# fnzhan/EMLight

Measured on AMD Instinct MI355X. Metric: training images/sec (regression step: DenseNet-BC fwd + Sinkhorn loss + bwd + Adam), higher is better.
Workload: dtype f32; 1 GPU; RegressionNetwork train step, BASELINE configs[1]; per_gpu_batch=64, global_batch=64, anchors=128, parallelism=single

## Files before the change

### emlight_amd/csrc/dense_bwd.hip

```cpp
#include "eml_common.h"
#include "eml_dropout.h"

#include <cstdint>
#include <cstdlib>
#include <type_traits>

namespace {

using f32x4 = __attribute__((ext_vector_type(4))) float;

__device__ __forceinline__ f32x4 mfma16(float a, float b, f32x4 c) {
  return __builtin_amdgcn_mfma_f32_16x16x4f32(a, b, c, 0, 0, 0);
}
__device__ __forceinline__ float f4c(const float4& v, int t) { return t == 0 ? v.x : t == 1 ? v.y : t == 2 ? v.z : v.w; }
__device__ __forceinline__ double shfl_xor_d(double v, int m) { return __shfl_xor(v, m, 64); }

constexpr int kTH = 8, kTW = 32, kHH = kTH + 2, kHW = kTW + 2;

constexpr int kPSG = 14;
constexpr int kBD = 512;
constexpr int kGRows = 2;
constexpr int kGPass = kHH / kGRows;

template <bool FUSE, bool WIDE, int TH, bool DROP = false>
// ... 1719 lines not shown
          const float4 c4 = *reinterpret_cast<const float4*>(co_l + 2 * Ko + ch);
          float4 dz[MT];
#pragma unroll
          for (int m = 0; m < MT; ++m) {
            dz[m].x = fmaf(a4.x, ry[m].x, fmaf(b4.x, rz[m].x, c4.x));
            dz[m].y = fmaf(a4.y, ry[m].y, fmaf(b4.y, rz[m].y, c4.y));
            dz[m].z = fmaf(a4.z, ry[m].z, fmaf(b4.z, rz[m].z, c4.z));
            dz[m].w = fmaf(a4.w, ry[m].w, fmaf(b4.w, rz[m].w, c4.w));
          }
          group_step(jo, dz);
        }
      }
      if constexpr (MASKED && !ACC) {
        float l1n[NCH][4];
        float4 skn[NCH];
#pragma unroll
        for (int n = 0; n < NCH; ++n) {
          skn[n] = *reinterpret_cast<const float4*>(vec_l + 16 * min(nt0 + n, nnt - 1) + 4 * kk);
#pragma unroll
          for (int g = 0; g < 4; ++g) l1n[n][g] = 0.f;
        }
        const int piece = lane & 7;
        const bool col_ok = nt0 + (piece >> 2) < nnt;
#pragma unroll
        for (int m = 0; m < MT; ++m) {
#pragma unroll
          for (int sub = 0; sub < 4; ++sub) {
#pragma unroll
            for (int n = 0; n < NCH; ++n) {
              const unsigned b = pv[m] ? mk[m][n] >> (4 * sub) : 0u;
              const float d0 = (b & 1u) ? 0.25f * acc[m][n][0] : 0.f, d1 = (b & 2u) ? 0.25f * acc[m][n][1] : 0.f;
              const float d2 = (b & 4u) ? 0.25f * acc[m][n][2] : 0.f, d3 = (b & 8u) ? 0.25f * acc[m][n][3] : 0.f;
              *reinterpret_cast<f32x4*>(stg + r * 36 + 16 * n + 4 * kk) = f32x4{skn[n].x * d0, skn[n].y * d1, skn[n].z * d2, skn[n].w * d3};
              if (nt0 + n < nnt) {
                l1n[n][0] += d0;
                l1n[n][1] += d1;
                l1n[n][2] += d2;
                l1n[n][3] += d3;
              }
            }
            __builtin_amdgcn_fence(__ATOMIC_RELEASE, "wavefront");
            __builtin_amdgcn_wave_barrier();
            __builtin_amdgcn_fence(__ATOMIC_ACQUIRE, "wavefront");
            const size_t suboff = ((size_t)(sub >> 1) * Win + (sub & 1)) * (size_t)ldg + 16 * nt0 + 4 * piece;
#pragma unroll
            for (int h = 0; h < 2; ++h) {
              const f32x4 v = *reinterpret_cast<const f32x4*>(stg + ((lane >> 3) + 8 * h) * 36 + 4 * piece);
              if (pvx[m][h] && col_ok) *reinterpret_cast<f32x4*>(Gd + pinx[m][h] * ldg + suboff) = v;
            }
            __builtin_amdgcn_fence(__ATOMIC_RELEASE, "wavefront");
            __builtin_amdgcn_wave_barrier();
            __builtin_amdgcn_fence(__ATOMIC_ACQUIRE, "wavefront");
          }
        }
#pragma unroll
        for (int n = 0; n < NCH; ++n) {
          if (nt0 + n < nnt) {
            const int k4 = 16 * (nt0 + n) + 4 * kk;
#pragma unroll
            for (int g = 0; g < 4; ++g) {
              const float t1 = eml::row16_sum(l1n[n][g]);
              if (r == 0) my[2 * (k4 + g)] += (double)t1;
            }
          }
        }
      } else {
#pragma unroll
      for (int n = 0; n < NCH; ++n) {
        const int nt = nt0 + n;
        if (nt < nnt) {
          const int k4 = 16 * nt + 4 * kk;
          const float4 sk = *reinterpret_cast<const float4*>(vec_l + k4);
          const float4 tk = *reinterpret_cast<const float4*>(vec_l + Kp + k4);
          const float4 mu = *reinterpret_cast<const float4*>(vec_l + 2 * Kp + k4);
          const float4 is = *reinterpret_cast<const float4*>(vec_l + 3 * Kp + k4);
          float l1[4] = {0.f, 0.f, 0.f, 0.f}, l2[4] = {0.f, 0.f, 0.f, 0.f};
#pragma unroll
          for (int m = 0; m < MT; ++m) {
            const float da0 = 0.25f * acc[m][n][0], da1 = 0.25f * acc[m][n][1];
            const float da2 = 0.25f * acc[m][n][2], da3 = 0.25f * acc[m][n][3];
#pragma unroll
            for (int sub = 0; sub < 4; ++sub) {
              float4 g = make_float4(0.f, 0.f, 0.f, 0.f);
              if constexpr (ACC) g = gs[m][n][sub];
              float d0, d1, d2, d3;
              float4 x = make_float4(0.f, 0.f, 0.f, 0.f);
              if constexpr (MASKED) {
                const unsigned b = pv[m] ? mk[m][n] >> (4 * sub) : 0u;
                d0 = (b & 1u) ? da0 : 0.f;
                d1 = (b & 2u) ? da1 : 0.f;
                d2 = (b & 4u) ? da2 : 0.f;
                d3 = (b & 8u) ? da3 : 0.f;
              } else {
                x = xv[m][n][sub];
                d0 = (pv[m] && fmaf(x.x, sk.x, tk.x) > 0.f) ? da0 : 0.f;
                d1 = (pv[m] && fmaf(x.y, sk.y, tk.y) > 0.f) ? da1 : 0.f;
                d2 = (pv[m] && fmaf(x.z, sk.z, tk.z) > 0.f) ? da2 : 0.f;
                d3 = (pv[m] && fmaf(x.w, sk.w, tk.w) > 0.f) ? da3 : 0.f;
              }
              g.x = fmaf(sk.x, d0, g.x);
              g.y = fmaf(sk.y, d1, g.y);
              g.z = fmaf(sk.z, d2, g.z);
              g.w = fmaf(sk.w, d3, g.w);
              if (pv[m]) {
                const size_t pi = pin[m] + (sub >> 1) * (size_t)Win + (sub & 1);
                *reinterpret_cast<float4*>(Gd + pi * ldg + k4) = g;
              }
              l1[0] += d0;
              l1[1] += d1;
              l1[2] += d2;
              l1[3] += d3;
              if constexpr (!MASKED) {
                l2[0] = fmaf(d0, (x.x - mu.x) * is.x, l2[0]);
                l2[1] = fmaf(d1, (x.y - mu.y) * is.y, l2[1]);
                l2[2] = fmaf(d2, (x.z - mu.z) * is.z, l2[2]);
                l2[3] = fmaf(d3, (x.w - mu.w) * is.w, l2[3]);
              }
            }
          }
#pragma unroll
          for (int g = 0; g < 4; ++g) {
            l1[g] = eml::row16_sum(l1[g]);
            if constexpr (!MASKED) l2[g] = eml::row16_sum(l2[g]);
            if (r == 0) {
              my[2 * (k4 + g)] += (double)l1[g];
              if constexpr (!MASKED) my[2 * (k4 + g) + 1] += (double)l2[g];
            }
          }
        }
      }
      }
    }
  }
  __syncthreads();
  for (int e = tid; e < Kp * 2; e += 256)
    partials[(size_t)blockIdx.x * Kp * 2 + e] =
        (sacc[e] + sacc[(size_t)Kp * 2 + e]) + (sacc[(size_t)2 * Kp * 2 + e] + sacc[(size_t)3 * Kp * 2 + e]);
}

struct BwdLayer {
  const float* DZ;
  const float* Zr;
  const float* cA;
  const float* cB;
  const float* cC;
  const float* Wd;
  const float* scale1;
  const float* shift1;
  double* partials;
  int Kp;
};

template <int NL, int MT , bool RAW = false ,
          bool MASKED = false, bool TOP = false>
__global__ __launch_bounds__(256, 2) void conv1x1_bwd_data_multi_kernel(BwdLayer L0, BwdLayer L1,
                                                                        const float* __restrict__ X, int ldx,
                                                                        const float* __restrict__ mean,
                                                                        const float* __restrict__ istd, int P,
                                                                        int k_lo, int k_hi, float* __restrict__ Gd,
                                                                        int ldg, int KpMax,
                                                                        const unsigned long long* __restrict__ M0,
                                                                        const unsigned long long* __restrict__ M1,
                                                                        float* __restrict__ Top) {
  extern __shared__ __attribute__((aligned(16))) float smem[];
  double* sacc = reinterpret_cast<double*>(smem);
  float* vec_l = reinterpret_cast<float*>(sacc + (size_t)NL * 4 * KpMax * 2);
  const int tid = threadIdx.x, lane = tid & 63, wave = tid >> 6;
  const int r = lane & 15, kk = lane >> 4;
  const BwdLayer Ls[2] = {L0, L1};
  for (int e = tid; e < NL * 4 * KpMax * 2; e += 256) sacc[e] = 0.0;
  for (int e = tid; e < KpMax; e += 256) {
    vec_l[e] = MASKED ? 0.f : mean[e];
    vec_l[KpMax + e] = MASKED ? 0.f : istd[e];
#pragma unroll
    for (int j = 0; j < NL; ++j) {
      vec_l[(2 + 2 * j) * KpMax + e] = e < Ls[j].Kp ? Ls[j].scale1[e] : 0.f;
      vec_l[(3 + 2 * j) * KpMax + e] = e < Ls[j].Kp ? Ls[j].shift1[e] : 0.f;
    }
  }
  __syncthreads();
  constexpr int TP = 64 * MT;
  const int ntiles = (P + TP - 1) / TP;
  const int nt_lo = k_lo >> 4, nt_hi = (k_hi + 15) >> 4;
  constexpr int NCH = 2;

  float4 wq[2][3][NCH];
  auto load_w = [&](int j, int nt0, float4 (&dst)[3][NCH]) {
    const int nnt = Ls[j].Kp >> 4;
#pragma unroll
    for (int jo = 0; jo < 3; ++jo)
#pragma unroll
      for (int n = 0; n < NCH; ++n) {
        const int nt = min(nt0 + n, nnt - 1);
        dst[jo][n] = *reinterpret_cast<const float4*>(Ls[j].Wd + ((((size_t)nt * 3 + jo) * 4 + kk) * 16 + r) * 4);
      }
  };
  load_w(0, nt_lo, wq[0]);
  int wsel = 0;

  for (int tile = blockIdx.x; tile < ntiles; tile += gridDim.x) {
    const int p0 = tile * TP + wave * 16 * MT;
    long prow[MT];
    bool pv[MT];
#pragma unroll
    for (int m = 0; m < MT; ++m) {
      pv[m] = p0 + 16 * m + r < P;
      prow[m] = min(p0 + 16 * m + r, P - 1);
    }
    unsigned long long pvb[MT];
#pragma unroll
    for (int m = 0; m < MT; ++m) pvb[m] = MASKED ? __ballot(pv[m]) : 0ull;
    float4 dz[NL][3][MT];
#pragma unroll
    for (int j = 0; j < NL; ++j)
#pragma unroll
      for (int jo = 0; jo < 3; ++jo) {
        const int ch = 16 * jo + 4 * kk;
        if constexpr (RAW) {
#pragma unroll
          for (int m = 0; m < MT; ++m) dz[j][jo][m] = *reinterpret_cast<const float4*>(Ls[j].DZ + prow[m] * 48 + ch);
        } else {
          const float4 a4 = *reinterpret_cast<const float4*>(Ls[j].cA + ch);
          const float4 b4 = *reinterpret_cast<const float4*>(Ls[j].cB + ch);
          const float4 c4 = *reinterpret_cast<const float4*>(Ls[j].cC + ch);
#pragma unroll
          for (int m = 0; m < MT; ++m) {
            const float4 dy = *reinterpret_cast<const float4*>(Ls[j].DZ + prow[m] * 48 + ch);
            const float4 zr = *reinterpret_cast<const float4*>(Ls[j].Zr + prow[m] * 48 + ch);
            dz[j][jo][m].x = fmaf(a4.x, dy.x, fmaf(b4.x, zr.x, c4.x));
            dz[j][jo][m].y = fmaf(a4.y, dy.y, fmaf(b4.y, zr.y, c4.y));
            dz[j][jo][m].z = fmaf(a4.z, dy.z, fmaf(b4.z, zr.z, c4.z));
            dz[j][jo][m].w = fmaf(a4.w, dy.w, fmaf(b4.w, zr.w, c4.w));
          }
        }
      }
    for (int nt0 = nt_lo; nt0 < nt_hi; nt0 += NCH) {
      float4 gs[MT][NCH], xv[MT][NCH];
#pragma unroll
      for (int n = 0; n < NCH; ++n) {
        const int k4 = 16 * min(nt0 + n, nt_hi - 1) + 4 * kk;
        const int k4l = (k4 + 3 >= k_lo && k4 < k_hi) ? k4 : (k_lo & ~3);
#pragma unroll
        for (int m = 0; m < MT; ++m) {
          gs[m][n] = *reinterpret_cast<const float4*>(Gd + prow[m] * ldg + k4l);
          if constexpr (!MASKED) xv[m][n] = *reinterpret_cast<const float4*>(X + prow[m] * ldx + k4l);
        }
      }
      const int nt_next = nt0 + NCH < nt_hi ? nt0 + NCH : nt_lo;
#pragma unroll
      for (int j = 0; j < NL; ++j) {
        const int nnt = Ls[j].Kp >> 4;
        unsigned long long mk[MT][NCH][4];
        if constexpr (MASKED) {
          const unsigned long long* __restrict__ Mj = j == 0 ? M0 : M1;
#pragma unroll
          for (int m = 0; m < MT; ++m)
#pragma unroll
            for (int n = 0; n < NCH; ++n) {
              const size_t wi =
                  ((size_t)__builtin_amdgcn_readfirstlane((p0 >> 4) + m) * nnt + min(nt0 + n, nnt - 1)) * 4;
#pragma unroll
              for (int g = 0; g < 4; ++g) mk[m][n][g] = Mj[wi + g];
            }
        }
        const int cur = NL == 2 ? j : wsel;
        if (j + 1 < NL)
          load_w(j + 1, nt0, wq[cur ^ 1]);
        else
          load_w(0, nt_next, wq[cur ^ 1]);
        __builtin_amdgcn_sched_barrier(0);
        f32x4 acc[MT][NCH];
#pragma unroll
        for (int m = 0; m < MT; ++m)
#pragma unroll
          for (int n = 0; n < NCH; ++n) acc[m][n] = f32x4{0.f, 0.f, 0.f, 0.f};
#pragma unroll
        for (int jo = 0; jo < 3; ++jo)
#pragma unroll
          for (int t = 0; t < 4; ++t)
#pragma unroll
            for (int n = 0; n < NCH; ++n)
#pragma unroll
              for (int m = 0; m < MT; ++m) acc[m][n] = mfma16(f4c(wq[cur][jo][n], t), f4c(dz[j][jo][m], t), acc[m][n]);
        if (NL == 1) wsel ^= 1;
        double* my = sacc + ((size_t)(j * 4 + wave) * KpMax) * 2;
#pragma unroll
        for (int n = 0; n < NCH; ++n) {
          const int nt = nt0 + n;
          if (nt < nnt && nt < nt_hi) {
            const int k4 = 16 * nt + 4 * kk;
            const float4 mu = *reinterpret_cast<const float4*>(vec_l + k4);
            const float4 is = *reinterpret_cast<const float4*>(vec_l + KpMax + k4);
            const float4 sk = *reinterpret_cast<const float4*>(vec_l + (2 + 2 * j) * KpMax + k4);
            const float4 tk = *reinterpret_cast<const float4*>(vec_l + (3 + 2 * j) * KpMax + k4);
            const bool in0 = k4 + 0 >= k_lo && k4 + 0 < k_hi, in1 = k4 + 1 >= k_lo && k4 + 1 < k_hi;
            const bool in2 = k4 + 2 >= k_lo && k4 + 2 < k_hi, in3 = k4 + 3 >= k_lo && k4 + 3 < k_hi;
            unsigned long long inb[4] = {0ull, 0ull, 0ull, 0ull};
            if constexpr (MASKED) {
              inb[0] = __ballot(in0);
              inb[1] = __ballot(in1);
              inb[2] = __ballot(in2);
              inb[3] = __ballot(in3);
            }
            float l1[4] = {0.f, 0.f, 0.f, 0.f}, l2[4] = {0.f, 0.f, 0.f, 0.f};
#pragma unroll
            for (int m = 0; m < MT; ++m) {
              float d0, d1, d2, d3;
              if constexpr (MASKED) {
                d0 = __builtin_amdgcn_inverse_ballot_w64(mk[m][n][0] & pvb[m] & inb[0]) ? acc[m][n][0] : 0.f;
                d1 = __builtin_amdgcn_inverse_ballot_w64(mk[m][n][1] & pvb[m] & inb[1]) ? acc[m][n][1] : 0.f;
                d2 = __builtin_amdgcn_inverse_ballot_w64(mk[m][n][2] & pvb[m] & inb[2]) ? acc[m][n][2] : 0.f;
                d3 = __builtin_amdgcn_inverse_ballot_w64(mk[m][n][3] & pvb[m] & inb[3]) ? acc[m][n][3] : 0.f;
              } else {
                const float4 x = xv[m][n];
                d0 = (pv[m] && in0 && fmaf(x.x, sk.x, tk.x) > 0.f) ? acc[m][n][0] : 0.f;
                d1 = (pv[m] && in1 && fmaf(x.y, sk.y, tk.y) > 0.f) ? acc[m][n][1] : 0.f;
                d2 = (pv[m] && in2 && fmaf(x.z, sk.z, tk.z) > 0.f) ? acc[m][n][2] : 0.f;
                d3 = (pv[m] && in3 && fmaf(x.w, sk.w, tk.w) > 0.f) ? acc[m][n][3] : 0.f;
                l2[0] = fmaf(d0, (x.x - mu.x) * is.x, l2[0]);
                l2[1] = fmaf(d1, (x.y - mu.y) * is.y, l2[1]);
                l2[2] = fmaf(d2, (x.z - mu.z) * is.z, l2[2]);
                l2[3] = fmaf(d3, (x.w - mu.w) * is.w, l2[3]);
              }
              gs[m][n].x = fmaf(sk.x, d0, gs[m][n].x);
              gs[m][n].y = fmaf(sk.y, d1, gs[m][n].y);
              gs[m][n].z = fmaf(sk.z, d2, gs[m][n].z);
              gs[m][n].w = fmaf(sk.w, d3, gs[m][n].w);
              l1[0] += d0;
              l1[1] += d1;
              l1[2] += d2;
              l1[3] += d3;
            }
#pragma unroll
            for (int g = 0; g < 4; ++g) {
              l1[g] = eml::row16_sum(l1[g]);
              if constexpr (!MASKED) l2[g] = eml::row16_sum(l2[g]);
              if (r == 0) {
                my[2 * (k4 + g)] += (double)l1[g];
                if constexpr (!MASKED) my[2 * (k4 + g) + 1] += (double)l2[g];
              }
            }
          }
        }
      }
#pragma unroll
      for (int n = 0; n < NCH; ++n) {
        const int nt = nt0 + n;
        if (nt < nt_hi) {
          const int k4 = 16 * nt + 4 * kk;
          const bool act = k4 + 3 >= k_lo && k4 < k_hi;
          if constexpr (TOP) {
            const int t = k4 - (k_hi - 24);
            float* cdst = Top + (t >= 12 ? (size_t)P * 12 + (t - 12) : (size_t)max(t, 0));
#pragma unroll
            for (int m = 0; m < MT; ++m) {
              float* dst = t >= 0 ? cdst + prow[m] * 12 : Gd + prow[m] * ldg + k4;
              if (pv[m] && act) *reinterpret_cast<float4*>(dst) = gs[m][n];
            }
          } else {
#pragma unroll
            for (int m = 0; m < MT; ++m) {
              if (pv[m] && act) *reinterpret_cast<float4*>(Gd + prow[m] * ldg + k4) = gs[m][n];
            }
          }
        }
      }
    }
  }
  __syncthreads();
#pragma unroll
  for (int j = 0; j < NL; ++j) {
    const int Kp = Ls[j].Kp;
    const double* base = sacc + (size_t)j * 4 * KpMax * 2;
    for (int e = tid; e < Kp * 2; e += 256)
      Ls[j].partials[(size_t)blockIdx.x * Kp * 2 + e] = (base[e] + base[(size_t)KpMax * 2 + e]) +
                                                        (base[(size_t)2 * KpMax * 2 + e] + base[(size_t)3 * KpMax * 2 + e]);
  }
}

template <int MT>
__global__ __launch_bounds__(256, 2) void conv1x1_bwd_narrow_kernel(
    const float* __restrict__ DZ, const float* __restrict__ W1 , int Cin, int k_lo,
    const float* __restrict__ X, int ldx, const float* __restrict__ scale1, const float* __restrict__ shift1,
    const float* __restrict__ mean, const float* __restrict__ istd, int P, const float* __restrict__ Gd, int ldg,
    float* __restrict__ N12, double* __restrict__ partials , int Kp) {
  __shared__ double red[4][12][2];
  const int tid = threadIdx.x, lane = tid & 63, wave = tid >> 6;
  const int r = lane & 15, kk = lane >> 4;
  float aw[3][4];
#pragma unroll
  for (int jo = 0; jo < 3; ++jo)
#pragma unroll
    for (int t = 0; t < 4; ++t) aw[jo][t] = r < 12 ? W1[(size_t)(16 * jo + 4 * kk + t) * Cin + k_lo + r] : 0.f;
  const bool cv = kk < 3;
  const int cq = k_lo + 4 * (cv ? kk : 2);
  float sk[4], tk[4], mu[4], is[4];
#pragma unroll
  for (int g = 0; g < 4; ++g) {
    sk[g] = scale1[cq + g];
    tk[g] = shift1[cq + g];
    mu[g] = mean[cq + g];
    is[g] = istd[cq + g];
  }
  double s1[4] = {0.0, 0.0, 0.0, 0.0}, s2[4] = {0.0, 0.0, 0.0, 0.0};
  constexpr int TP = 64 * MT;
  const int ntiles = (P + TP - 1) / TP;
  for (int tile = blockIdx.x; tile < ntiles; tile += gridDim.x) {
    const int p0 = tile * TP + wave * 16 * MT;
    size_t prow[MT];
    bool pv[MT];
    float4 dz[MT][3];
    float2 xa[MT], xb[MT], ga[MT], gb[MT];
#pragma unroll
    for (int m = 0; m < MT; ++m) {
      pv[m] = p0 + 16 * m + r < P;
      prow[m] = (size_t)min(p0 + 16 * m + r, P - 1);
#pragma unroll
      for (int jo = 0; jo < 3; ++jo) dz[m][jo] = *reinterpret_cast<const float4*>(DZ + prow[m] * 48 + 16 * jo + 4 * kk);
      xa[m] = *reinterpret_cast<const float2*>(X + prow[m] * ldx + cq);
      xb[m] = *reinterpret_cast<const float2*>(X + prow[m] * ldx + cq + 2);
      ga[m] = *reinterpret_cast<const float2*>(Gd + prow[m] * ldg + cq);
      gb[m] = *reinterpret_cast<const float2*>(Gd + prow[m] * ldg + cq + 2);
    }
    f32x4 acc[MT];
#pragma unroll
    for (int m = 0; m < MT; ++m) acc[m] = f32x4{0.f, 0.f, 0.f, 0.f};
#pragma unroll
    for (int jo = 0; jo < 3; ++jo)
#pragma unroll
      for (int t = 0; t < 4; ++t)
#pragma unroll
        for (int m = 0; m < MT; ++m) acc[m] = mfma16(aw[jo][t], f4c(dz[m][jo], t), acc[m]);
#pragma unroll
    for (int m = 0; m < MT; ++m) {
      const float x[4] = {xa[m].x, xa[m].y, xb[m].x, xb[m].y};
      const float gold[4] = {ga[m].x, ga[m].y, gb[m].x, gb[m].y};
      float o[4];
#pragma unroll
      for (int g = 0; g < 4; ++g) {
        const float d = (pv[m] && cv && fmaf(x[g], sk[g], tk[g]) > 0.f) ? acc[m][g] : 0.f;
        o[g] = fmaf(sk[g], d, gold[g]);
        s1[g] += (double)d;
        s2[g] += (double)(d * ((x[g] - mu[g]) * is[g]));
      }
      if (pv[m] && cv) *reinterpret_cast<float4*>(N12 + prow[m] * 12 + 4 * kk) = make_float4(o[0], o[1], o[2], o[3]);
    }
  }
#pragma unroll
  for (int g = 0; g < 4; ++g) {
#pragma unroll
    for (int o = 1; o < 16; o <<= 1) {
      s1[g] += shfl_xor_d(s1[g], o);
      s2[g] += shfl_xor_d(s2[g], o);
    }
    if (r == 0 && cv) {
      red[wave][4 * kk + g][0] = s1[g];
      red[wave][4 * kk + g][1] = s2[g];
    }
  }
  __syncthreads();
  if (tid < 24) {
    const int c = tid >> 1, e = tid & 1;
    partials[((size_t)blockIdx.x * Kp + k_lo + c) * 2 + e] = (red[0][c][e] + red[1][c][e]) + (red[2][c][e] + red[3][c][e]);
  }
}

__global__ void permute_w1_bwd_kernel(const float* __restrict__ W, int Cout, int Cin, int Kp, int Ko,
                                      float* __restrict__ Wd) {
  const size_t total = (size_t)Kp * Ko;
  for (size_t e = (size_t)blockIdx.x * blockDim.x + threadIdx.x; e < total; e += (size_t)gridDim.x * blockDim.x) {
    const int t = (int)(e & 3), col = (int)((e >> 2) & 15), kk = (int)((e >> 6) & 3);
    const size_t rest = e >> 8;
    const int jo = (int)(rest % (Ko >> 4)), nt = (int)(rest / (Ko >> 4));
    const int o = 16 * jo + 4 * kk + t, k = 16 * nt + col;
    Wd[e] = (o < Cout && k < Cin) ? W[(size_t)o * Cin + k] : 0.f;
  }
}

__global__ __launch_bounds__(256) void grad_materialize_kernel(float* __restrict__ Gd, int ldg,
                                                               const float* __restrict__ X, int ldx,
                                                               const float* __restrict__ sB,
                                                               const float* __restrict__ sC, int c0, int n, size_t P) {
  const int nh = n >> 1;
  const size_t total = P * nh;
  for (size_t e = (size_t)blockIdx.x * 256 + threadIdx.x; e < total; e += (size_t)gridDim.x * 256) {
    const size_t p = e / nh;
    const int c = c0 + 2 * (int)(e - p * nh);
    const float2 x = *reinterpret_cast<const float2*>(X + p * ldx + c);
    float2* gp = reinterpret_cast<float2*>(Gd + p * ldg + c);
    float2 g = *gp;
    g.x += fmaf(sB[c], x.x, sC[c]);
    g.y += fmaf(sB[c + 1], x.y, sC[c + 1]);
    *gp = g;
// ... 695 lines not shown
extern "C" int eml_dense_conv1x1_bwd_weight_f32(const float* X, int ldx, long P, int Hin, int Win, int pool, int Kp,
                                                int Cin, const float* scale1, const float* shift1, const float* DY,
                                                int ld_dy, const float* Zr, int ld_z, const float* cA, const float* cB,
                                                const float* cC, int Cout, float* partial, float* dW, int grid,
                                                float* dz_out, const float* W1, int k_lo, const float* G, int ldg,
                                                float* N12, double* partials_n, eml_stream_t stream) {
  if (dz_out && (Cout != 48 || pool))
    return eml::fail(EML_EINVAL, "eml_dense_conv1x1_bwd_weight_f32: dz_out is for dense layers (Cout == 48, no pool)");
  if (N12 && (Cout != 48 || pool || !W1 || !G || !partials_n || k_lo < 0 || (k_lo & 1) || k_lo + 12 > Cin || (ldg & 1) ||
              (ldg != 12 && k_lo + 12 > ldg)))
    return eml::fail(EML_EINVAL, "eml_dense_conv1x1_bwd_weight_f32: fused narrow pass needs a dense layer, W1, G, partials_n "
                                 "and an even k_lo with k_lo + 12 <= Cin (k_lo=%d, Cin=%d)", k_lo, Cin);
  if (!X || !scale1 || !shift1 || !DY || !Zr || !cA || !cB || !cC || !partial || !dW || P < 1 || grid < 1 || Kp < 32 ||
      (Kp & 15) || Cin > Kp || Cout < 1)
    return eml::fail(EML_EINVAL, "eml_dense_conv1x1_bwd_weight_f32: bad arguments");
  const int nchunks = (Cout + 47) / 48;
  for (int ch = 0; ch < nchunks; ++ch) {
    const int n0 = ch * 48, nv = (Cout - n0 < 48) ? Cout - n0 : 48;
    int n_load = ((ld_dy < ld_z ? ld_dy : ld_z) - n0) & ~3;
    if (n_load > 48) n_load = 48;
    if (n_load < nv) return eml::fail(EML_EINVAL, "eml_dense_conv1x1_bwd_weight_f32: DY/Zr rows narrower than Cout");
    const NarrowArgs na{W1, G, N12, partials_n, Cin, k_lo, ldg};
    static const int vec_env = [] { const char* v = getenv("EML_W1_VEC"); return v ? atoi(v) : 0; }();
    const bool vec4 = !pool && (ldx & 3) == 0 && (reinterpret_cast<uintptr_t>(X) & 15) == 0 &&
                      vec_env == 4;
    if (vec4 && N12 && vec_env == 4)
      hipLaunchKernelGGL((conv1x1_bwd_weight_kernel<false, true, 4>), dim3(grid), dim3(256), 0, (hipStream_t)stream, X, ldx,
                         (int)P, Hin, Win, Kp, scale1, shift1, DY + n0, ld_dy, Zr + n0, ld_z, cA + n0, cB + n0, cC + n0,
                         nv, n_load, partial, dz_out, na);
    else if (vec4 && !N12)
      hipLaunchKernelGGL((conv1x1_bwd_weight_kernel<false, false, 4>), dim3(grid), dim3(256), 0, (hipStream_t)stream, X, ldx,
                         (int)P, Hin, Win, Kp, scale1, shift1, DY + n0, ld_dy, Zr + n0, ld_z, cA + n0, cB + n0, cC + n0,
                         nv, n_load, partial, dz_out, na);
    else if (pool)
      hipLaunchKernelGGL((conv1x1_bwd_weight_kernel<true, false>), dim3(grid), dim3(256), 0, (hipStream_t)stream, X, ldx,
                         (int)P, Hin, Win, Kp, scale1, shift1, DY + n0, ld_dy, Zr + n0, ld_z, cA + n0, cB + n0, cC + n0,
                         nv, n_load, partial, nullptr, na);
    else if (N12)
      hipLaunchKernelGGL((conv1x1_bwd_weight_kernel<false, true>), dim3(grid), dim3(256), 0, (hipStream_t)stream, X, ldx,
                         (int)P, Hin, Win, Kp, scale1, shift1, DY + n0, ld_dy, Zr + n0, ld_z, cA + n0, cB + n0, cC + n0,
                         nv, n_load, partial, dz_out, na);
    else
      hipLaunchKernelGGL((conv1x1_bwd_weight_kernel<false, false>), dim3(grid), dim3(256), 0, (hipStream_t)stream, X, ldx,
                         (int)P, Hin, Win, Kp, scale1, shift1, DY + n0, ld_dy, Zr + n0, ld_z, cA + n0, cB + n0, cC + n0,
                         nv, n_load, partial, dz_out, na);
    int rc = eml::check_launch("eml_dense_conv1x1_bwd_weight_f32");
    if (rc) return rc;
    hipLaunchKernelGGL(reduce_rows_kernel, dim3((Cin * 48 + 63) / 64), dim3(256), 0, (hipStream_t)stream, partial,
                       grid, (size_t)Kp * 48, 0, Cin, nv, n0, dW);
    rc = eml::check_launch("eml_dense_conv1x1_bwd_weight_f32(reduce)");
    if (rc) return rc;
  }
  return EML_OK;
}

extern "C" int eml_dense_permute_w1_bwd_f32(const float* W, int Cout, int Cin, int Kp, int Ko, float* Wd,
                                            eml_stream_t stream) {
  if (!W || !Wd || Cout < 1 || Cin < 1 || Kp < Cin || (Kp & 15) || Ko < Cout || (Ko & 15))
    return eml::fail(EML_EINVAL, "eml_dense_permute_w1_bwd_f32: bad arguments");
  hipLaunchKernelGGL(permute_w1_bwd_kernel, dim3(64), dim3(256), 0, (hipStream_t)stream, W, Cout, Cin, Kp, Ko, Wd);
  return eml::check_launch("eml_dense_permute_w1_bwd_f32");
}

extern "C" int eml_dense_conv1x1_bwd_data_f32(const float* DY, int ld_dy, const float* Zr, int ld_z, const float* cA,
                                              const float* cB, const float* cC, int Ko, const float* Wd,
                                              const float* X, int ldx, const float* scale1, const float* shift1,
                                              const float* mean, const float* istd, long P, int Hin, int Win, int pool,
                                              int Kp, float* G, int ldg, int accumulate, double* partials, int grid,
                                              const unsigned short* relu_mask16, eml_stream_t stream) {
  if (!DY || !Zr || !cA || !cB || !cC || !Wd || (!relu_mask16 && (!X || !mean || !istd)) || !scale1 || !shift1 || !G ||
      !partials || P < 1 || grid < 1 || (Kp & 15) || (Ko & 15) || Ko > ld_dy || Ko > ld_z || (ld_dy & 3) || (ld_z & 3) ||
      (ldx & 3) || (ldg & 3) || (!relu_mask16 && Kp > ldx) || Kp > ldg)
    return eml::fail(EML_EINVAL, "eml_dense_conv1x1_bwd_data_f32: bad arguments");
  if (relu_mask16 && !(pool && Ko != 48))
    return eml::fail(EML_EINVAL, "eml_dense_conv1x1_bwd_data_f32: relu_mask16 is for the transition form (pool, Ko != 48)");
  const size_t lds = (size_t)4 * Kp * 2 * sizeof(double);
#define EML_LAUNCH_BWD_DATA(POOLV, RESV, NCHV)                                                                        \
  hipLaunchKernelGGL((conv1x1_bwd_data_kernel<POOLV, RESV, NCHV>), dim3(grid), dim3(256), lds, (hipStream_t)stream, DY, \
                     ld_dy, Zr, ld_z, cA, cB, cC, Ko, Wd, X, ldx, scale1, shift1, mean, istd, (int)P, Hin, Win, Kp, G, \
                     ldg, accumulate, partials)
  if (pool) {
    if (Ko == 48) {
      EML_LAUNCH_BWD_DATA(true, true, 4);
    } else {
      const size_t lds_t = lds + (size_t)(4 * Kp + 3 * Ko + 4 * 16 * 36) * sizeof(float);
#define EML_LAUNCH_TRANSITION(ACCV, MSKV)                                                                              \
  do {                                                                                                                \
    EML_ENSURE_LDS((&transition_bwd_data_kernel<2, 2, ACCV, MSKV>), lds_t);                                 \
    hipLaunchKernelGGL((transition_bwd_data_kernel<2, 2, ACCV, MSKV>), dim3(grid), dim3(256), lds_t,                   \
                       (hipStream_t)stream, DY, ld_dy, Zr, ld_z, cA, cB, cC, Ko, Wd, X, ldx, scale1, shift1, mean, istd, \
                       (int)P, Hin, Win, Kp, G, ldg, partials, relu_mask16);                                           \
  } while (0)
#define EML_LAUNCH_TRANSITION_RES(NJOV)                                                                                \
  do {                                                                                                                \
    EML_ENSURE_LDS((&transition_bwd_data_kernel<2, 2, false, true, NJOV>), lds_t);                                     \
    hipLaunchKernelGGL((transition_bwd_data_kernel<2, 2, false, true, NJOV>), dim3(grid), dim3(256), lds_t,            \
                       (hipStream_t)stream, DY, ld_dy, Zr, ld_z, cA, cB, cC, Ko, Wd, X, ldx, scale1, shift1, mean, istd, \
                       (int)P, Hin, Win, Kp, G, ldg, partials, relu_mask16);                                           \
  } while (0)
      if (relu_mask16 && !accumulate && Ko == 112) EML_LAUNCH_TRANSITION_RES(7);
      else if (relu_mask16 && !accumulate && Ko == 160) EML_LAUNCH_TRANSITION_RES(10);
      else if (relu_mask16 && !accumulate && Ko == 176) EML_LAUNCH_TRANSITION_RES(11);
      else if (relu_mask16) {
        if (accumulate) EML_LAUNCH_TRANSITION(true, true); else EML_LAUNCH_TRANSITION(false, true);
      } else {
        if (accumulate) EML_LAUNCH_TRANSITION(true, false); else EML_LAUNCH_TRANSITION(false, false);
      }
#undef EML_LAUNCH_TRANSITION
#undef EML_LAUNCH_TRANSITION_RES
    }
  } else {
    if (Ko == 48) EML_LAUNCH_BWD_DATA(false, true, 2); else EML_LAUNCH_BWD_DATA(false, false, 4);
  }
#undef EML_LAUNCH_BWD_DATA
  return eml::check_launch("eml_dense_conv1x1_bwd_data_f32");
}

namespace {
int launch_bwd_data_multi(int n_layers, const float* const* DZ, const float* const* Zr, const float* const* cA,
                          const float* const* cB, const float* const* cC, const float* const* Wd,
                          const float* const* scale1, const float* const* shift1, double* const* partials, const int* Kp,
                          const float* X, int ldx, const float* mean, const float* istd, long P, int k_lo, int k_hi,
                          float* G, int ldg, int grid, const unsigned long long* const* relu_masks, float* top,
                          eml_stream_t stream) {
  if (top && (n_layers != 2 || !relu_masks || Zr || k_lo != 0 || k_hi < 24 || (k_hi & 3) || P * 12 > 2147483647L))
    return eml::fail(EML_EINVAL, "eml_dense_conv1x1_bwd_data_multi_top_f32: the compact top-24 output needs two layers, "
                                 "relu_masks, materialised dz, k_lo == 0 and k_hi >= 24, a multiple of 4 (k_hi=%d)", k_hi);
  if (n_layers < 1 || n_layers > 2 || !DZ || !Wd || !scale1 || !shift1 || !partials ||
      !Kp || (!relu_masks && (!X || !mean || !istd)) || !G || P < 1 || grid < 1 || k_lo < 0 || k_hi <= k_lo ||
      (ldx & 3) || (ldg & 3))
    return eml::fail(EML_EINVAL, "eml_dense_conv1x1_bwd_data_multi_f32: bad arguments");
  const bool raw = Zr == nullptr;
  if (!raw && (!cA || !cB || !cC))
    return eml::fail(EML_EINVAL, "eml_dense_conv1x1_bwd_data_multi_f32: Zr given without cA/cB/cC");
  if (relu_masks && !raw)
    return eml::fail(EML_EINVAL, "eml_dense_conv1x1_bwd_data_multi_f32: relu_masks needs the materialised dz (Zr == NULL)");
  BwdLayer L[2];
  const unsigned long long* Mk[2] = {nullptr, nullptr};
  int kmax = 0;
  for (int j = 0; j < 2; ++j) {
    const int s = j < n_layers ? j : 0;
    const unsigned long long* mk = relu_masks ? relu_masks[s] : nullptr;
    Mk[j] = mk;
    L[j] = raw ? BwdLayer{DZ[s], nullptr, nullptr, nullptr, nullptr, Wd[s], scale1[s], shift1[s], partials[s], Kp[s]}
               : BwdLayer{DZ[s], Zr[s], cA[s], cB[s], cC[s], Wd[s], scale1[s], shift1[s], partials[s], Kp[s]};
    if (!DZ[s] || (!raw && !Zr[s]) || !Wd[s] || !partials[s] || (relu_masks && !mk) || (Kp[s] & 15) ||
        (!relu_masks && Kp[s] > ldx) || Kp[s] > ldg)
      return eml::fail(EML_EINVAL, "eml_dense_conv1x1_bwd_data_multi_f32: bad layer %d", s);
    if (Kp[s] > kmax) kmax = Kp[s];
  }
  if (((k_hi + 15) & ~15) > kmax) return eml::fail(EML_EINVAL, "eml_dense_conv1x1_bwd_data_multi_f32: range beyond Kp");
  const size_t lds = (size_t)n_layers * 4 * kmax * 2 * sizeof(double) + (size_t)(2 + 2 * n_layers) * kmax * sizeof(float);
  if (lds > 80 * 1024) return eml::fail(EML_EINVAL, "eml_dense_conv1x1_bwd_data_multi_f32: Kp=%d does not fit LDS", kmax);
#define EML_LAUNCH_MULTI(NLV, MTV, RAWV, MSKV)                                                                       \
  do {                                                                                                              \
    EML_ENSURE_LDS((&conv1x1_bwd_data_multi_kernel<NLV, MTV, RAWV, MSKV>), lds);                                 \
    hipLaunchKernelGGL((conv1x1_bwd_data_multi_kernel<NLV, MTV, RAWV, MSKV>), dim3(grid), dim3(256), lds,            \
                       (hipStream_t)stream, L[0], L[1], X, ldx, mean, istd, (int)P, k_lo, k_hi, G, ldg, kmax,        \
                       Mk[0], Mk[1], (float*)nullptr);                                                              \
  } while (0)
  if (n_layers == 1) {
    if (relu_masks) EML_LAUNCH_MULTI(1, 4, true, true);
    else if (raw) EML_LAUNCH_MULTI(1, 4, true, false);
    else EML_LAUNCH_MULTI(1, 4, false, false);
  } else if (top) {
    EML_ENSURE_LDS((&conv1x1_bwd_data_multi_kernel<2, 2, true, true, true>), lds);
    hipLaunchKernelGGL((conv1x1_bwd_data_multi_kernel<2, 2, true, true, true>), dim3(grid), dim3(256), lds,
                       (hipStream_t)stream, L[0], L[1], X, ldx, mean, istd, (int)P, k_lo, k_hi, G, ldg, kmax, Mk[0], Mk[1],
                       top);
  } else {
    if (relu_masks) EML_LAUNCH_MULTI(2, 2, true, true);
    else if (raw) EML_LAUNCH_MULTI(2, 2, true, false);
    else EML_LAUNCH_MULTI(2, 2, false, false);
  }
#undef EML_LAUNCH_MULTI
  return eml::check_launch("eml_dense_conv1x1_bwd_data_multi_f32");
}
}

extern "C" int eml_dense_conv1x1_bwd_data_multi_f32(int n_layers, const float* const* DZ, const float* const* Zr,
                                                    const float* const* cA, const float* const* cB,
                                                    const float* const* cC, const float* const* Wd,
                                                    const float* const* scale1, const float* const* shift1,
                                                    double* const* partials, const int* Kp, const float* X, int ldx,
                                                    const float* mean, const float* istd, long P, int k_lo, int k_hi,
                                                    float* G, int ldg, int grid,
                                                    const unsigned long long* const* relu_masks, eml_stream_t stream) {
  return launch_bwd_data_multi(n_layers, DZ, Zr, cA, cB, cC, Wd, scale1, shift1, partials, Kp, X, ldx, mean, istd, P, k_lo,
                               k_hi, G, ldg, grid, relu_masks, nullptr, stream);
}

extern "C" int eml_dense_conv1x1_bwd_data_multi_top_f32(const float* const* DZ, const float* const* Wd,
                                                        const float* const* scale1, const float* const* shift1,
                                                        double* const* partials, const int* Kp, long P, int k_hi,
                                                        float* G, int ldg, int grid,
                                                        const unsigned long long* const* relu_masks, float* top,
                                                        eml_stream_t stream) {
  if (!top) return eml::fail(EML_EINVAL, "eml_dense_conv1x1_bwd_data_multi_top_f32: top is NULL");
  return launch_bwd_data_multi(2, DZ, nullptr, nullptr, nullptr, nullptr, Wd, scale1, shift1, partials, Kp, nullptr, 0,
                               nullptr, nullptr, P, 0, k_hi, G, ldg, grid, relu_masks, top, stream);
}

extern "C" int eml_dense_conv1x1_bwd_narrow_f32(const float* DZ, const float* W1, int Cin, int k_lo, const float* X,
                                                int ldx, const float* scale1, const float* shift1, const float* mean,
                                                const float* istd, long P, const float* G, int ldg, float* N12,
                                                double* partials, int Kp, int grid, eml_stream_t stream) {
  if (!DZ || !W1 || !X || !scale1 || !shift1 || !mean || !istd || !G || !N12 || !partials || P < 1 || grid < 1 ||
      k_lo < 0 || (k_lo & 1) || k_lo + 12 > Cin || Cin > Kp || (ldx & 1) || (ldg & 1) || Kp > ldx || Kp > ldg)
    return eml::fail(EML_EINVAL, "eml_dense_conv1x1_bwd_narrow_f32: bad arguments");
  hipLaunchKernelGGL((conv1x1_bwd_narrow_kernel<4>), dim3(grid), dim3(256), 0, (hipStream_t)stream, DZ, W1, Cin, k_lo, X,
                     ldx, scale1, shift1, mean, istd, (int)P, G, ldg, N12, partials, Kp);
  return eml::check_launch("eml_dense_conv1x1_bwd_narrow_f32");
}

extern "C" int eml_dense_grad_materialize_f32(float* G, int ldg, const float* X, int ldx, const float* sB,
                                              const float* sC, int c0, int n, long P, eml_stream_t stream) {
  if (!G || !X || !sB || !sC || P < 1 || n < 2 || (n & 1) || (c0 & 1) || (ldg & 1) || (ldx & 1))
    return eml::fail(EML_EINVAL, "eml_dense_grad_materialize_f32: bad arguments");
  const size_t total = (size_t)P * (n >> 1);
  const int grid = (int)((total + 255) / 256 < 8192 ? (total + 255) / 256 : 8192);
  hipLaunchKernelGGL(grad_materialize_kernel, dim3(grid), dim3(256), 0, (hipStream_t)stream, G, ldg, X, ldx, sB, sC, c0,
                     n, (size_t)P);
  return eml::check_launch("eml_dense_grad_materialize_f32");
}

extern "C" int eml_dense_bn_bwd_stats_f32(const float* DY, int ld_dy, const float* raw, int ld_raw, const float* out,
                                          int ld_out, int relu, int C, long P, const float* mean, const float* istd,
                                          double* partials, int grid, eml_stream_t stream) {
  if (!DY || !raw || !mean || !istd || !partials || (relu && !out) || C < 1 || C > 384 || P < 1 || grid < 1)
    return eml::fail(EML_EINVAL, "eml_dense_bn_bwd_stats_f32: bad arguments");
  auto a16 = [](const void* q) { return (reinterpret_cast<size_t>(q) & 15) == 0; };
  if (C <= 32 && (C & 3) == 0 && ((ld_dy | ld_raw | (relu ? ld_out : 0)) & 3) == 0 && a16(DY) && a16(raw) && (!relu || a16(out)) &&
      a16(mean) && a16(istd)) {
    hipLaunchKernelGGL(bn_bwd_stats_small_kernel, dim3(grid), dim3(256), 0, (hipStream_t)stream, DY, ld_dy, raw, ld_raw, out, ld_out,
                       relu, C, (size_t)P, mean, istd, partials);
    return eml::check_launch("eml_dense_bn_bwd_stats_f32");
  }
  const size_t lds = (size_t)4 * ((C + 63) / 64) * 64 * 2 * sizeof(double);
  hipLaunchKernelGGL(bn_bwd_stats_kernel, dim3(grid), dim3(256), lds, (hipStream_t)stream, DY, ld_dy, raw, ld_raw, out,
                     ld_out, relu, C, (size_t)P, mean, istd, partials);
  return eml::check_launch("eml_dense_bn_bwd_stats_f32");
}

extern "C" int eml_dense_conv0_bwd_weight_f32(const float* x, const float* G, int ldg, const float* X1, int ldx,
                                              const float* Y0, int C0, const float* cA, const float* cB,
                                              const float* cC, int B, int H, int W, float* partial, float* dW0,
                                              int grid, eml_stream_t stream) {
  if (!x || !G || !X1 || !Y0 || !cA || !cB || !cC || !partial || !dW0 || C0 < 1 || C0 > 32 || B < 1 || grid < 1)
    return eml::fail(EML_EINVAL, "eml_dense_conv0_bwd_weight_f32: bad arguments");
  hipLaunchKernelGGL(conv0_bwd_weight_kernel<false>, dim3(grid), dim3(256), 0, (hipStream_t)stream, x, G, ldg, X1, ldx, Y0, C0,
                     cA, cB, cC, B, H, W, partial, nullptr, nullptr, nullptr, nullptr);
  int rc = eml::check_launch("eml_dense_conv0_bwd_weight_f32");
  if (rc) return rc;
  hipLaunchKernelGGL(reduce_rows_kernel, dim3(27 * 32 / 64 + 1), dim3(256), 0, (hipStream_t)stream, partial, grid * 4,
                     (size_t)1024, 2, 0, C0, 0, dW0);
  return eml::check_launch("eml_dense_conv0_bwd_weight_f32(reduce)");
}

extern "C" int eml_dense_head_pool_bwd_f32(const float* gpooled, const float* F, int ldf, int C, int B, int H, int W,
                                           int k, float* dF, int ldd, eml_stream_t stream) {
  if (!gpooled || !F || !dF || C < 1 || B < 1 || k < 1) return eml::fail(EML_EINVAL, "eml_dense_head_pool_bwd_f32: bad arguments");
  const size_t total = (size_t)B * H * W * C;
  const int grid = (int)((total + 255) / 256 < 4096 ? (total + 255) / 256 : 4096);
  hipLaunchKernelGGL(head_pool_bwd_kernel, dim3(grid), dim3(256), 0, (hipStream_t)stream, gpooled, F, ldf, C, B, H, W, k,
                     dF, ldd);
  return eml::check_launch("eml_dense_head_pool_bwd_f32");
}

extern "C" int eml_dense_norm0_bwd_stats_f32(const float* G, int ldg, const float* Y0, int ld_y0, const float* scale0,
                                             const float* shift0, const float* sB, const float* sC, int C, long P,
                                             const float* mean, const float* istd, double* partials, int grid,
                                             eml_stream_t stream) {
  auto a16 = [](const void* q) { return (reinterpret_cast<size_t>(q) & 15) == 0; };
  if (!G || !Y0 || !scale0 || !shift0 || !sB || !sC || !mean || !istd || !partials || C < 4 || C > 32 || (C & 3) || P < 1 ||
      grid < 1 || ((ldg | ld_y0) & 3) || !a16(G) || !a16(Y0) || !a16(scale0) || !a16(shift0) || !a16(sB) || !a16(sC) || !a16(mean) ||
      !a16(istd))
    return eml::fail(EML_EINVAL, "eml_dense_norm0_bwd_stats_f32: bad arguments (C a multiple of 4 <= 32, 16-byte aligned operands)");
  hipLaunchKernelGGL(norm0_bwd_stats_kernel, dim3(grid), dim3(256), 0, (hipStream_t)stream, G, ldg, Y0, ld_y0, scale0, shift0, sB,
                     sC, C, (size_t)P, mean, istd, partials);
  return eml::check_launch("eml_dense_norm0_bwd_stats_f32");
}

extern "C" int eml_dense_conv0_bwd_weight_fused_f32(const float* x, const float* G, int ldg, const float* Y0, int C0,
                                                    const float* scale0, const float* shift0, const float* sB, const float* sC,
                                                    const float* cA, const float* cB, const float* cC, int B, int H, int W,
                                                    float* partial, float* dW0, int grid, eml_stream_t stream) {
  if (!x || !G || !Y0 || !scale0 || !shift0 || !sB || !sC || !cA || !cB || !cC || !partial || !dW0 || C0 < 1 || C0 > 32 || B < 1 ||
      grid < 1)
    return eml::fail(EML_EINVAL, "eml_dense_conv0_bwd_weight_fused_f32: bad arguments");
  hipLaunchKernelGGL(conv0_bwd_weight_kernel<true>, dim3(grid), dim3(256), 0, (hipStream_t)stream, x, G, ldg, nullptr, 0, Y0, C0, cA,
                     cB, cC, B, H, W, partial, scale0, shift0, sB, sC);
  int rc = eml::check_launch("eml_dense_conv0_bwd_weight_fused_f32");
  if (rc) return rc;
  hipLaunchKernelGGL(reduce_rows_kernel, dim3(27 * 32 / 64 + 1), dim3(256), 0, (hipStream_t)stream, partial, grid * 4,
                     (size_t)1024, 2, 0, C0, 0, dW0);
  return eml::check_launch("eml_dense_conv0_bwd_weight_fused_f32(reduce)");
}

extern "C" int eml_dense_conv0_bwd_data_f32(const float* G, int ldg, const float* X1, int ldx, const float* Y0, int C0,
                                            const float* scale0, const float* shift0, const float* sB, const float* sC,
                                            const float* cA, const float* cB, const float* cC, const float* W0, int B, int H,
                                            int W, float* dX, eml_stream_t stream) {
  auto a16 = [](const void* q) { return (reinterpret_cast<size_t>(q) & 15) == 0; };
  const bool fused = X1 == nullptr;
  if (!G || !Y0 || !cA || !cB || !cC || !W0 || !dX || (fused && (!scale0 || !shift0 || !sB || !sC)))
    return eml::fail(EML_EINVAL, "eml_dense_conv0_bwd_data_f32: null pointer");
  if (C0 != kC0dC || B < 1 || H < 1 || W < 1 || ldg < C0 || (ldg & 3) || (!fused && (ldx < C0 || (ldx & 3))))
    return eml::fail(EML_EINVAL, "eml_dense_conv0_bwd_data_f32: bad shape (C0 == 24, B, H, W >= 1, ldg / ldx >= 24 and multiples of 4)");
  if (!a16(G) || !a16(Y0) || (!fused && !a16(X1)) || !a16(cA) || !a16(cB) || !a16(cC) ||
      (fused && (!a16(scale0) || !a16(shift0) || !a16(sB) || !a16(sC))))
    return eml::fail(EML_EINVAL, "eml_dense_conv0_bwd_data_f32: G, X1, Y0 and the coefficient vectors must be 16-byte aligned");
  const size_t tiles = (size_t)B * ((H + kC0dTH - 1) / kC0dTH) * ((W + kC0dTW - 1) / kC0dTW);
  if (tiles > 0x7fffffff) return eml::fail(EML_EINVAL, "eml_dense_conv0_bwd_data_f32: more than 2^31 - 1 tiles of 8 x 32 pixels");
  const int grid = (int)tiles;
  if (fused)
    hipLaunchKernelGGL(conv0_bwd_data_kernel<true>, dim3(grid), dim3(256), 0, (hipStream_t)stream, G, ldg, nullptr, 0, Y0,
                       scale0, shift0, sB, sC, cA, cB, cC, W0, B, H, W, dX);
  else
    hipLaunchKernelGGL(conv0_bwd_data_kernel<false>, dim3(grid), dim3(256), 0, (hipStream_t)stream, G, ldg, X1, ldx, Y0,
                       nullptr, nullptr, nullptr, nullptr, cA, cB, cC, W0, B, H, W, dX);
  return eml::check_launch("eml_dense_conv0_bwd_data_f32");
}
```

Baseline: 569.6 images/s.

## Batch dgrad epilogue reductions and preload ReLU masks with lane-distributed loads

Adds an EPI template mode to the multi-layer 1x1 backward-data kernel, selected through the EML_DGRAD_EPI environment variable and defaulting to 2. In this mode one lane-distributed load fetches all ReLU mask words and readlane broadcasts them, replacing many per-wave scalar loads. The per-column row16 reductions are gathered so each of several lanes owns one accumulator slot and writes it, instead of lane 0 doing every write, and the LDS old value and scale vectors are prefetched before the MFMA block. Mode 2 also skips the second N-chunk's MFMAs when that chunk is out of range. This adds register pressure and more template instances, and relies on static_asserts about the mask layout.

```diff
diff --git a/emlight_amd/csrc/dense_bwd.hip b/emlight_amd/csrc/dense_bwd.hip
--- a/emlight_amd/csrc/dense_bwd.hip
+++ b/emlight_amd/csrc/dense_bwd.hip
@@ -1895,7 +1895,7 @@
 };
 
 template <int NL, int MT , bool RAW = false ,
-          bool MASKED = false, bool TOP = false>
+          bool MASKED = false, bool TOP = false, int EPI = 0>
 __global__ __launch_bounds__(256, 2) void conv1x1_bwd_data_multi_kernel(BwdLayer L0, BwdLayer L1,
                                                                         const float* __restrict__ X, int ldx,
                                                                         const float* __restrict__ mean,
@@ -1941,6 +1941,13 @@
   load_w(0, nt_lo, wq[0]);
   int wsel = 0;
 
+  auto mask_word = [&](int pg , int c0) {
+    static_assert(!MASKED || NL * MT * NCH * 4 == 32, "one ballot word per lane of a half wave");
+    const int li = lane & 31, mj = li / (MT * NCH * 4), mm = (li >> 3) & (MT - 1), mn = (li >> 2) & 1, mg = li & 3;
+    const int mnnt = (mj ? L1.Kp : L0.Kp) >> 4;
+    return (mj ? M1 : M0)[((size_t)(pg + mm) * mnnt + min(c0 + mn, mnnt - 1)) * 4 + mg];
+  };
+
   for (int tile = blockIdx.x; tile < ntiles; tile += gridDim.x) {
     const int p0 = tile * TP + wave * 16 * MT;
     long prow[MT];
@@ -1989,12 +1996,14 @@
           if constexpr (!MASKED) xv[m][n] = *reinterpret_cast<const float4*>(X + prow[m] * ldx + k4l);
         }
       }
+      unsigned long long mv = 0ull;
+      if constexpr (EPI && MASKED) mv = mask_word(p0 >> 4, nt0);
       const int nt_next = nt0 + NCH < nt_hi ? nt0 + NCH : nt_lo;
 #pragma unroll
       for (int j = 0; j < NL; ++j) {
         const int nnt = Ls[j].Kp >> 4;
         unsigned long long mk[MT][NCH][4];
-        if constexpr (MASKED) {
+        if constexpr (MASKED && !EPI) {
           const unsigned long long* __restrict__ Mj = j == 0 ? M0 : M1;
 #pragma unroll
           for (int m = 0; m < MT; ++m)
@@ -2011,22 +2020,60 @@
           load_w(j + 1, nt0, wq[cur ^ 1]);
         else
           load_w(0, nt_next, wq[cur ^ 1]);
+        double* my = sacc + ((size_t)(j * 4 + wave) * KpMax) * 2;
+        const int own_nt = nt0 + ((r >> 2) & 1);
+        const bool own = r < 8 && own_nt < nnt && own_nt < nt_hi;
+        double* slot = my + 2 * (16 * own_nt + 4 * kk + (r & 3));
+        double old1 = 0.0;
+        float4 skq[NCH];
+        if constexpr (EPI && MASKED) {
+          old1 = slot[0];
+#pragma unroll
+          for (int n = 0; n < NCH; ++n)
+            skq[n] = *reinterpret_cast<const float4*>(vec_l + (2 + 2 * j) * KpMax + 16 * min(nt0 + n, nt_hi - 1) + 4 * kk);
+        }
         __builtin_amdgcn_sched_barrier(0);
         f32x4 acc[MT][NCH];
 #pragma unroll
         for (int m = 0; m < MT; ++m)
 #pragma unroll
           for (int n = 0; n < NCH; ++n) acc[m][n] = f32x4{0.f, 0.f, 0.f, 0.f};
-#pragma unroll
-        for (int jo = 0; jo < 3; ++jo)
-#pragma unroll
-          for (int t = 0; t < 4; ++t)
+        if (EPI < 2 || (nt0 + 1 < nnt && nt0 + 1 < nt_hi)) {
+#pragma unroll
+          for (int jo = 0; jo < 3; ++jo)
+#pragma unroll
+            for (int t = 0; t < 4; ++t)
+#pragma unroll
+              for (int n = 0; n < NCH; ++n)
+#pragma unroll
+                for (int m = 0; m < MT; ++m) acc[m][n] = mfma16(f4c(wq[cur][jo][n], t), f4c(dz[j][jo][m], t), acc[m][n]);
+        } else {
+#pragma unroll
+          for (int jo = 0; jo < 3; ++jo)
+#pragma unroll
+            for (int t = 0; t < 4; ++t)
+#pragma unroll
+              for (int m = 0; m < MT; ++m) acc[m][0] = mfma16(f4c(wq[cur][jo][0], t), f4c(dz[j][jo][m], t), acc[m][0]);
+        }
+        if (NL == 1) wsel ^= 1;
+        if constexpr (EPI && MASKED) {
+          __builtin_amdgcn_sched_barrier(0);
+#pragma unroll
+          for (int m = 0; m < MT; ++m)
 #pragma unroll
             for (int n = 0; n < NCH; ++n)
 #pragma unroll
-              for (int m = 0; m < MT; ++m) acc[m][n] = mfma16(f4c(wq[cur][jo][n], t), f4c(dz[j][jo][m], t), acc[m][n]);
-        if (NL == 1) wsel ^= 1;
-        double* my = sacc + ((size_t)(j * 4 + wave) * KpMax) * 2;
+              for (int g = 0; g < 4; ++g) {
+                const int w = ((j * MT + m) * NCH + n) * 4 + g;
+                mk[m][n][g] = (unsigned long long)(unsigned)__builtin_amdgcn_readlane((int)mv, w) |
+                              (unsigned long long)(unsigned)__builtin_amdgcn_readlane((int)(mv >> 32), w) << 32;
+              }
+        }
+        float l1n[NCH][4], l2n[NCH][4];
+#pragma unroll
+        for (int n = 0; n < NCH; ++n)
+#pragma unroll
+          for (int g = 0; g < 4; ++g) l1n[n][g] = l2n[n][g] = 0.f;
 #pragma unroll
         for (int n = 0; n < NCH; ++n) {
           const int nt = nt0 + n;
@@ -2034,7 +2081,9 @@
             const int k4 = 16 * nt + 4 * kk;
             const float4 mu = *reinterpret_cast<const float4*>(vec_l + k4);
             const float4 is = *reinterpret_cast<const float4*>(vec_l + KpMax + k4);
-            const float4 sk = *reinterpret_cast<const float4*>(vec_l + (2 + 2 * j) * KpMax + k4);
+            float4 sk;
+            if constexpr (EPI && MASKED) sk = skq[n];
+            else sk = *reinterpret_cast<const float4*>(vec_l + (2 + 2 * j) * KpMax + k4);
             const float4 tk = *reinterpret_cast<const float4*>(vec_l + (3 + 2 * j) * KpMax + k4);
             const bool in0 = k4 + 0 >= k_lo && k4 + 0 < k_hi, in1 = k4 + 1 >= k_lo && k4 + 1 < k_hi;
             const bool in2 = k4 + 2 >= k_lo && k4 + 2 < k_hi, in3 = k4 + 3 >= k_lo && k4 + 3 < k_hi;
@@ -2074,14 +2123,46 @@
               l1[2] += d2;
               l1[3] += d3;
             }
-#pragma unroll
-            for (int g = 0; g < 4; ++g) {
-              l1[g] = eml::row16_sum(l1[g]);
-              if constexpr (!MASKED) l2[g] = eml::row16_sum(l2[g]);
-              if (r == 0) {
-                my[2 * (k4 + g)] += (double)l1[g];
-                if constexpr (!MASKED) my[2 * (k4 + g) + 1] += (double)l2[g];
+            if constexpr (EPI) {
+#pragma unroll
+              for (int g = 0; g < 4; ++g) {
+                l1n[n][g] = l1[g];
+                l2n[n][g] = l2[g];
               }
+            } else {
+#pragma unroll
+              for (int g = 0; g < 4; ++g) {
+                l1[g] = eml::row16_sum(l1[g]);
+                if constexpr (!MASKED) l2[g] = eml::row16_sum(l2[g]);
+                if (r == 0) {
+                  my[2 * (k4 + g)] += (double)l1[g];
+                  if constexpr (!MASKED) my[2 * (k4 + g) + 1] += (double)l2[g];
+                }
+              }
+            }
+          }
+        }
+        if constexpr (EPI) {
+          const bool b0 = r & 1, b1 = r & 2, b2 = r & 4;
+          auto pick4 = [&](const float (&s)[4]) {
+            const float s0 = eml::row16_sum(s[0]), s1 = eml::row16_sum(s[1]);
+            const float s2 = eml::row16_sum(s[2]), s3 = eml::row16_sum(s[3]);
+            return b1 ? (b0 ? s3 : s2) : (b0 ? s1 : s0);
+          };
+          auto pick = [&](const float (&s)[NCH][4]) {
+            static_assert(NCH == 2, "tile r >> 2 of two");
+            const float q0 = pick4(s[0]), q1 = pick4(s[1]);
+            return b2 ? q1 : q0;
+          };
+          const float v1 = pick(l1n);
+          float v2 = 0.f;
+          if constexpr (!MASKED) v2 = pick(l2n);
+          if (own) {
+            if constexpr (MASKED) {
+              slot[0] = old1 + (double)v1;
+            } else {
+              slot[0] += (double)v1;
+              slot[1] += (double)v2;
             }
           }
         }
@@ -3083,27 +3164,34 @@
   if (((k_hi + 15) & ~15) > kmax) return eml::fail(EML_EINVAL, "eml_dense_conv1x1_bwd_data_multi_f32: range beyond Kp");
   const size_t lds = (size_t)n_layers * 4 * kmax * 2 * sizeof(double) + (size_t)(2 + 2 * n_layers) * kmax * sizeof(float);
   if (lds > 80 * 1024) return eml::fail(EML_EINVAL, "eml_dense_conv1x1_bwd_data_multi_f32: Kp=%d does not fit LDS", kmax);
-#define EML_LAUNCH_MULTI(NLV, MTV, RAWV, MSKV)                                                                       \
+  const char* epi_env = getenv("EML_DGRAD_EPI");
+  const int epi = epi_env && epi_env[0] >= '0' && epi_env[0] <= '2' && !epi_env[1] ? epi_env[0] - '0' : 2;
+#define EML_LAUNCH_MULTI_E(NLV, MTV, RAWV, MSKV, TOPV, EPIV)                                                         \
   do {                                                                                                              \
-    EML_ENSURE_LDS((&conv1x1_bwd_data_multi_kernel<NLV, MTV, RAWV, MSKV>), lds);                                 \
-    hipLaunchKernelGGL((conv1x1_bwd_data_multi_kernel<NLV, MTV, RAWV, MSKV>), dim3(grid), dim3(256), lds,            \
+    EML_ENSURE_LDS((&conv1x1_bwd_data_multi_kernel<NLV, MTV, RAWV, MSKV, TOPV, EPIV>), lds);                         \
+    hipLaunchKernelGGL((conv1x1_bwd_data_multi_kernel<NLV, MTV, RAWV, MSKV, TOPV, EPIV>), dim3(grid), dim3(256), lds, \
                        (hipStream_t)stream, L[0], L[1], X, ldx, mean, istd, (int)P, k_lo, k_hi, G, ldg, kmax,        \
-                       Mk[0], Mk[1], (float*)nullptr);                                                              \
+                       Mk[0], Mk[1], top);                                                                          \
+  } while (0)
+#define EML_LAUNCH_MULTI(NLV, MTV, RAWV, MSKV, TOPV)                                                                 \
+  do {                                                                                                              \
+    if (epi == 0) EML_LAUNCH_MULTI_E(NLV, MTV, RAWV, MSKV, TOPV, 0);                                                 \
+    else if (epi == 1) EML_LAUNCH_MULTI_E(NLV, MTV, RAWV, MSKV, TOPV, 1);                                            \
+    else EML_LAUNCH_MULTI_E(NLV, MTV, RAWV, MSKV, TOPV, 2);                                                          \
   } while (0)
   if (n_layers == 1) {
-    if (relu_masks) EML_LAUNCH_MULTI(1, 4, true, true);
-    else if (raw) EML_LAUNCH_MULTI(1, 4, true, false);
-    else EML_LAUNCH_MULTI(1, 4, false, false);
+    if (relu_masks) EML_LAUNCH_MULTI(1, 4, true, true, false);
+    else if (raw) EML_LAUNCH_MULTI(1, 4, true, false, false);
+    else EML_LAUNCH_MULTI(1, 4, false, false, false);
   } else if (top) {
-    EML_ENSURE_LDS((&conv1x1_bwd_data_multi_kernel<2, 2, true, true, true>), lds);
-    hipLaunchKernelGGL((conv1x1_bwd_data_multi_kernel<2, 2, true, true, true>), dim3(grid), dim3(256), lds,
-                       (hipStream_t)stream, L[0], L[1], X, ldx, mean, istd, (int)P, k_lo, k_hi, G, ldg, kmax, Mk[0], Mk[1],
-                       top);
+    EML_LAUNCH_MULTI(2, 2, true, true, true);
   } else {
-    if (relu_masks) EML_LAUNCH_MULTI(2, 2, true, true);
-    else if (raw) EML_LAUNCH_MULTI(2, 2, true, false);
-    else EML_LAUNCH_MULTI(2, 2, false, false);
-  }
+    if (relu_masks) EML_LAUNCH_MULTI(2, 2, true, true, false);
+    else if (raw) EML_LAUNCH_MULTI(2, 2, true, false, false);
+    else if (epi == 0) EML_LAUNCH_MULTI_E(2, 2, false, false, false, 0);
+    else EML_LAUNCH_MULTI_E(2, 2, false, false, false, 1);
+  }
+#undef EML_LAUNCH_MULTI_E
 #undef EML_LAUNCH_MULTI
   return eml::check_launch("eml_dense_conv1x1_bwd_data_multi_f32");
 }
```

New measurement: 573.8 images/s (median of 6 runs). Within noise of the previous version (+0.7%).
